# DavidHan008/SLAM-1

Measured on AMD Instinct MI355X. Metric: frames/sec tracking+local-BA @1280x720, higher is better.
Workload: dtype u8+f32+f64

## Files before the change

### include/slam355.h

```cpp
#ifndef SLAM355_H
#define SLAM355_H

#include <stddef.h>
#include <stdint.h>

#ifdef __cplusplus
extern "C" {
#endif

#define SLAM355_ABI_VERSION 1

#define SLAM_OK 0
#define SLAM_ERR_ARG (-1)
#define SLAM_ERR_HIP (-2)
#define SLAM_ERR_WORKSPACE (-3)
#define SLAM_ERR_COMM (-4)

int slam_abi_version(void);
const char* slam_last_error(void);
int slam_device_count(void);

int slam_hamming_knn2(const uint8_t* d_q, const int32_t* d_nq, int q_cap,
                      const uint8_t* d_t, const int32_t* d_nt, int t_cap,
                      int batch, int32_t* d_idx2, int32_t* d_dist2,
                      uint8_t* d_good, void* stream);

int slam_hamming_force_valu(int valu);

int slam_compact_matches(const int32_t* d_idx2, const uint8_t* d_good,
                         const int32_t* d_nq, int q_cap, int batch,
                         const double* d_gate_xyz, double gate,
                         int32_t* d_pairs, int32_t* d_count, void* stream);



int slam_gather_matches(const float* d_kpq, int kq_cap, const float* d_kpt, int kt_cap,
                        const uint8_t* d_desq, const uint8_t* d_dest, const int32_t* d_pairs,
                        const int32_t* d_count, int p_cap, int batch, double* d_ptq,
                        double* d_ptt, uint8_t* d_dq, uint8_t* d_dt, void* stream);

int slam_gather_temporal(const double* d_X, const double* d_ptl, int xcap, const float* d_kp_next,
                         int kcap, const int32_t* d_pairs, const int32_t* d_count, int pcap,
                         int batch, double* d_Q1, double* d_q2, double* d_q1, void* stream);

int slam_fundamental_lmeds(const double* d_m1, const double* d_m2, const int32_t* d_count,
                           int cap, int batch, uint64_t seed, int item0, int n_hyp,
                           uint8_t* d_mask, double* d_F, int32_t* d_ninliers, void* stream);

int slam_filter_pairs(const int32_t* d_pairs, const int32_t* d_count, const uint8_t* d_mask,
                      int cap, int batch, int32_t* d_out, int32_t* d_out_count, void* stream);

int slam_triangulate(const double* d_ptl, const double* d_ptr, const int32_t* d_count, int cap,
                     int batch, const double* d_Pl, const double* d_Pr, int proj_stride,
                     double* d_X, void* stream);

int slam_pnp_ransac(const double* d_Q, const double* d_q, const int32_t* d_count, int cap,
                    int batch, const double* d_K, uint64_t seed, int item0, int n_hyp,
                    double reproj_thresh, int hyp_iters, int refine_iters, double* d_rvec,
                    double* d_tvec, int32_t* d_ninliers, uint8_t* d_mask, double* d_ws,
                    long long ws_len, void* stream);
long long slam_pnp_workspace_len(int batch, int n_hyp);

int slam_pose_chain(const double* d_rvec, const double* d_tvec, const int32_t* d_ninliers,
                    int batch, double* d_state, double* d_poses, void* stream);

int slam_vo_estimate_pose(const double* d_q1, const double* d_q2, const double* d_Q1,
                          const double* d_Q2, const int32_t* d_count, int cap, int batch,
                          const double* d_P, uint64_t seed, int item0, int max_iter,
                          int lm_iters, int early_stop, double* d_pose, int32_t* d_best,
                          int32_t* d_ntried, double* d_err, void* d_ws, size_t ws_bytes,
                          void* stream);
int slam_vo_pose_workspace_bytes(int batch, int max_iter, size_t* bytes);

int slam_vo_residuals(const double* d_dof, const double* d_q1, const double* d_q2,
                      const double* d_Q1, const double* d_Q2, const int32_t* d_count, int cap,
                      int batch, const double* d_P, double* d_res, void* stream);

int slam_rel_to_abs(const double* d_rel, const int32_t* d_count, int cap, int batch,
                    const double* d_poses, double* d_abs, void* stream);

int slam_map_workspace_bytes(int max_queries, int map_cap, size_t* bytes);
int slam_map_associate(double* d_map, int32_t* d_M, int map_cap, int M_bound,
                       const double* d_abs, const double* d_rel, const double* d_pts2d,
                       const int32_t* d_n, int N, double threshold, int frame_index,
                       double* d_rows, void* d_ws, size_t ws_size, void* stream);
int slam_map_windows(double* d_maps, int32_t* d_M, int map_cap, int n_win, int n,
                     const double* d_abs, const double* d_rel, const double* d_pts2d,
                     const int32_t* d_count, int cap, double threshold, double* d_rows,
                     void* d_ws, size_t ws_size, void* stream);

int slam_orb_workspace_bytes(int batch, int H, int W, int max_kp, int overlap_div,
                             int height_div, int width_div, size_t* bytes);
int slam_orb_tiles(const uint8_t* d_img, int batch, int H, int W, int stride, int max_kp,
                   int overlap_div, int height_div, int width_div, void* d_ws,
                   size_t ws_bytes, float* d_kp, int32_t* d_octave, uint8_t* d_desc,
                   int32_t* d_count, int kp_cap, void* stream);


int slam_ba_residual(const double* d_cams, const double* d_pts, const int32_t* d_cam_idx,
                     const int32_t* d_pt_idx, const double* d_qs, int n_obs,
// ... 194 lines not shown
```

### slam-1_amd/csrc/fundamental.hip

```cpp
#include "common.hpp"

#include <cmath>

namespace {

#ifndef SLAM_FMH_WG
#define SLAM_FMH_WG 256
#endif
constexpr int kHWG = SLAM_FMH_WG, kHWaves = kHWG / 64;
constexpr int kFWG = 64;
constexpr int kS = 7;

__device__ inline uint64_t splitmix64(uint64_t& s) {
  s += 0x9E3779B97F4A7C15ull;
  uint64_t z = s;
  z = (z ^ (z >> 30)) * 0xBF58476D1CE4E5B9ull;
  z = (z ^ (z >> 27)) * 0x94D049BB133111EBull;
  return z ^ (z >> 31);
}

__device__ __forceinline__ void draw_sample(uint64_t& s, int M, int idx[kS]) {
#pragma unroll
  for (int k = 0; k < kS; ++k) {
    int v;
// ... 188 lines not shown
  const double cc2 = (v1 + vm) / 2.0 - cc0;
  const double s = (v1 - vm) / 2.0;
  const double u = v2 - 4.0 * cc2 - cc0;
  const double cc3 = (u - 2.0 * s) / 6.0;
  const double cc1 = s - cc3;
  double roots[3];
  const int nr = cubic_roots(cc3, cc2, cc1, cc0, roots);
  const double T1[9] = {s1, 0, -s1 * c1x, 0, s1, -s1 * c1y, 0, 0, 1};
  const double T2[9] = {s2, 0, -s2 * c2x, 0, s2, -s2 * c2y, 0, 0, 1};
  int n = 0;
#pragma unroll
  for (int k = 0; k < 3; ++k) {
    if (k >= nr) break;
    double Fn[9], tmp[9], F[9];
#pragma unroll
    for (int i = 0; i < 9; ++i) Fn[i] = roots[k] * F1[i] + (1.0 - roots[k]) * F2[i];
#pragma unroll
    for (int i = 0; i < 3; ++i)
#pragma unroll
      for (int j = 0; j < 3; ++j)
        tmp[3 * i + j] = Fn[3 * i] * T1[j] + Fn[3 * i + 1] * T1[3 + j] + Fn[3 * i + 2] * T1[6 + j];
#pragma unroll
    for (int i = 0; i < 3; ++i)
#pragma unroll
      for (int j = 0; j < 3; ++j)
        F[3 * i + j] = T2[i] * tmp[j] + T2[3 + i] * tmp[3 + j] + T2[6 + i] * tmp[6 + j];
    double nrm = 0.0;
#pragma unroll
    for (int i = 0; i < 9; ++i) nrm += F[i] * F[i];
    nrm = sqrt(nrm);
    if (!(nrm > 0.0) || !isfinite(nrm)) continue;
#pragma unroll
    for (int i = 0; i < 9; ++i) out[n][i] = F[i] / nrm;
    ++n;
  }
  return n;
}

__device__ __forceinline__ float fm_error(const double* F, const double* p1, const double* p2) {
  double a = F[0] * p1[0] + F[1] * p1[1] + F[2];
  double b = F[3] * p1[0] + F[4] * p1[1] + F[5];
  double c = F[6] * p1[0] + F[7] * p1[1] + F[8];
  const double s2 = 1.0 / (a * a + b * b);
  const double d2 = p2[0] * a + p2[1] * b + c;
  a = F[0] * p2[0] + F[3] * p2[1] + F[6];
  b = F[1] * p2[0] + F[4] * p2[1] + F[7];
  c = F[2] * p2[0] + F[5] * p2[1] + F[8];
  const double s1 = 1.0 / (a * a + b * b);
  const double d1 = p1[0] * a + p1[1] * b + c;
  const float e = (float)fmax(d1 * d1 * s1, d2 * d2 * s2);
  return isnan(e) ? INFINITY : e;
}

constexpr int kSplit = 8;
constexpr int kRound = 64;
constexpr int kEv = 12;
static_assert(kSplit * 8 <= 9 * 8, "per-split bests must fit F[b]");
#ifdef SLAM_FMH_TRACE
__device__ unsigned long long g_fmh[8];
#define FMH_T(i) do { if (threadIdx.x == 0 && blockIdx.x == 3 && blockIdx.y == 5) g_fmh[i] = __builtin_amdgcn_s_memtime(); } while (0)
#else
#define FMH_T(i) (void)0
#endif

__global__ __launch_bounds__(kHWG) void k_fm_hyp(const double* __restrict__ m1all,
                                                const double* __restrict__ m2all,
                                                const int32_t* __restrict__ count, int cap,
                                                uint64_t seed, int item0, int n_hyp,
                                                double* __restrict__ Fout) {
  __shared__ double cand[kRound][3][9];
  __shared__ int ncand[kRound];
  __shared__ int hist[kHWaves][256];
  __shared__ float wbest[kHWaves];
  __shared__ int wbidx[kHWaves];
  const int b = blockIdx.x, sp = blockIdx.y, t = threadIdx.x;
  const int lane = t & 63, w = t >> 6;
  const int M = min(max(count[b], 0), cap);
  if (M < 8) return;
  const double* m1 = m1all + (size_t)b * cap * 2;
  const double* m2 = m2all + (size_t)b * cap * 2;
  const int hb = (int)((long long)n_hyp * sp / kSplit), he = (int)((long long)n_hyp * (sp + 1) / kSplit);
  float my_best = INFINITY;
  int my_idx = 0x7FFFFFFF;
  const int need = M / 2 + 1;
  FMH_T(0);
#ifdef SLAM_FMH_TRACE
  int n_sel = 0, n_cand = 0;
#endif
  for (int h0 = hb; h0 < he; h0 += kRound) {
    const int nh = min(kRound, he - h0);
    __syncthreads();
    if (t < nh) {
      const int h = h0 + t;
      uint64_t s = seed ^ ((uint64_t)(item0 + b) * 0xD1B54A32D192ED03ull) ^
                   ((uint64_t)h * 0x9FB21C651E98DF25ull);
      int idx[kS];
      draw_sample(s, M, idx);
      ncand[t] = seven_point(m1, m2, idx, cand[t]);
    }
    __syncthreads();
    FMH_T(1);
    int ln = lane;
    asm volatile("" : "+v"(ln));
    double pc[kEv][4];
#pragma unroll
    for (int j = 0; j < kEv; ++j) {
      const int i = min(ln + 64 * j, M - 1);
      pc[j][0] = m1[2 * i];
      pc[j][1] = m1[2 * i + 1];
      pc[j][2] = m2[2 * i];
      pc[j][3] = m2[2 * i + 1];
    }
    for (int hl = w; hl < nh; hl += kHWaves) {
      for (int k = 0; k < ncand[hl]; ++k) {
        const double* F = cand[hl][k];
        int below = 0;
        float ev[kEv];
#pragma unroll
        for (int j = 0; j < kEv; ++j) {
          ev[j] = INFINITY;
          if (ln + 64 * j < M) {
            ev[j] = fm_error(F, pc[j], pc[j] + 2);
            below += ev[j] < my_best ? 1 : 0;
          }
        }
        for (int i = ln + 64 * kEv; i < M; i += 64)
          below += fm_error(F, m1 + 2 * i, m2 + 2 * i) < my_best ? 1 : 0;
        for (int off = 32; off > 0; off >>= 1) below += __shfl_xor(below, off, 64);
#ifdef SLAM_FMH_TRACE
        ++n_cand;
#endif
        if (below < need) continue;
#ifdef SLAM_FMH_TRACE
        ++n_sel;
#endif
        uint32_t prefix = 0, pmask = 0;
        int krank = M / 2;
        for (int shift = 24; shift >= 0; shift -= 8) {
          for (int j = lane; j < 256; j += 64) hist[w][j] = 0;
          __builtin_amdgcn_wave_barrier();
#pragma unroll
          for (int j = 0; j < kEv; ++j) {
            const uint32_t bits = __float_as_uint(ev[j]);
            if (ln + 64 * j < M && (bits & pmask) == prefix)
              atomicAdd(&hist[w][(bits >> shift) & 255u], 1);
          }
          for (int i = ln + 64 * kEv; i < M; i += 64) {
            const uint32_t bits = __float_as_uint(fm_error(F, m1 + 2 * i, m2 + 2 * i));
            if ((bits & pmask) == prefix) atomicAdd(&hist[w][(bits >> shift) & 255u], 1);
          }
          __builtin_amdgcn_wave_barrier();
          __builtin_amdgcn_s_waitcnt(0xC07F);
          const int c0 = hist[w][4 * lane], c1 = hist[w][4 * lane + 1];
          const int c2 = hist[w][4 * lane + 2], c3 = hist[w][4 * lane + 3];
          const int sm = c0 + c1 + c2 + c3;
          int inc = sm;
          for (int off = 1; off < 64; off <<= 1) {
            const int o = __shfl_up(inc, off, 64);
            if (lane >= off) inc += o;
          }
          const int exc = inc - sm;
          int bin = -1, before = 0;
          if (krank >= exc && krank < inc) {
            int acc = exc;
            if (krank < acc + c0) { bin = 4 * lane; before = acc; }
            else if (krank < acc + c0 + c1) { bin = 4 * lane + 1; before = acc + c0; }
            else if (krank < acc + c0 + c1 + c2) { bin = 4 * lane + 2; before = acc + c0 + c1; }
            else { bin = 4 * lane + 3; before = acc + c0 + c1 + c2; }
          }
          const unsigned long long bal = __ballot(bin >= 0);
          const int src = __ffsll((long long)bal) - 1;
          bin = __shfl(bin, src, 64);
          before = __shfl(before, src, 64);
          krank -= before;
          prefix |= (uint32_t)bin << shift;
          pmask |= 255u << shift;
        }
        const float med = __uint_as_float(prefix);
        if (med < my_best) {
          my_best = med;
          my_idx = (h0 + hl) * 3 + k;
        }
      }
    }
  }
  FMH_T(2);
#ifdef SLAM_FMH_TRACE
  if (threadIdx.x == 0 && blockIdx.x == 3 && blockIdx.y == 5) { g_fmh[5] = n_cand; g_fmh[6] = n_sel; g_fmh[7] = M; }
#endif
  if (lane == 0) {
    wbest[w] = my_best;
    wbidx[w] = my_idx;
  }
  __syncthreads();
  FMH_T(3);
  if (t == 0) {
    float bm = INFINITY;
    int bi = 0x7FFFFFFF;
    for (int i = 0; i < kHWaves; ++i)
      if (wbest[i] < bm || (wbest[i] == bm && wbidx[i] < bi)) {
        bm = wbest[i];
        bi = wbidx[i];
      }
    float* slot = reinterpret_cast<float*>(Fout + 9 * (size_t)b) + 2 * sp;
    slot[0] = bm;
    reinterpret_cast<int*>(slot)[1] = bi;
  }
}

__global__ __launch_bounds__(kFWG) void k_fm_finish(const double* __restrict__ m1all,
                                                   const double* __restrict__ m2all,
                                                   const int32_t* __restrict__ count, int cap,
                                                   uint64_t seed, int item0,
                                                   uint8_t* __restrict__ mask,
                                                   double* __restrict__ Fout,
                                                   int32_t* __restrict__ ninl) {
  __shared__ double Fb[9];
  __shared__ double Fw[3][9];
  __shared__ float best_s;
  __shared__ int found_s, cnt_s;
  const int b = blockIdx.x, t = threadIdx.x;
  const int lane = t & 63;
  const int M = min(max(count[b], 0), cap);
  const double* m1 = m1all + (size_t)b * cap * 2;
  const double* m2 = m2all + (size_t)b * cap * 2;
  uint8_t* mk = mask + (size_t)b * cap;
  if (M < 8) {
    for (int i = t; i < M; i += kFWG) mk[i] = 0;
    if (t < 9) Fout[9 * b + t] = 0.0;
    if (t == 0) ninl[b] = -1;
    return;
  }
  if (t == 0) {
    const float* slots = reinterpret_cast<const float*>(Fout + 9 * (size_t)b);
    float bm = INFINITY;
    int bi = 0x7FFFFFFF;
    for (int i = 0; i < kSplit; ++i) {
      const float v = slots[2 * i];
      const int ix = reinterpret_cast<const int*>(slots)[2 * i + 1];
      if (v < bm || (v == bm && ix < bi)) {
        bm = v;
        bi = ix;
      }
    }
    best_s = bm;
    found_s = bi != 0x7FFFFFFF && bm < INFINITY;
    cnt_s = 0;
    if (found_s) {
      const int h = bi / 3, k = bi % 3;
      uint64_t s = seed ^ ((uint64_t)(item0 + b) * 0xD1B54A32D192ED03ull) ^
                   ((uint64_t)h * 0x9FB21C651E98DF25ull);
      int idx[kS];
      draw_sample(s, M, idx);
      seven_point(m1, m2, idx, Fw);
      for (int i = 0; i < 9; ++i) Fb[i] = Fw[k][i];
    }
  }
  __syncthreads();
  if (!found_s) {
    for (int i = t; i < M; i += kFWG) mk[i] = 0;
    if (t < 9) Fout[9 * b + t] = 0.0;
    if (t == 0) ninl[b] = -1;
    return;
  }
  double sigma = 2.5 * 1.4826 * (1 + 5.0 / (M - kS)) * sqrt((double)best_s);
  sigma = fmax(sigma, 0.001);
  const double thr = sigma * sigma;
  double F[9];
  for (int i = 0; i < 9; ++i) F[i] = Fb[i];
  int c = 0;
  for (int i = t; i < M; i += kFWG) {
    const uint8_t in = (double)fm_error(F, m1 + 2 * i, m2 + 2 * i) <= thr ? 1 : 0;
    mk[i] = in;
    c += in;
  }
  for (int off = 32; off > 0; off >>= 1) c += __shfl_xor(c, off, 64);
  if (lane == 0) atomicAdd(&cnt_s, c);
  __syncthreads();
  if (t < 9) Fout[9 * b + t] = F[t];
  if (t == 0) ninl[b] = cnt_s;
}

#ifndef SLAM_CWG
#define SLAM_CWG 1024
#endif
constexpr int kCWG = SLAM_CWG;
__global__ __launch_bounds__(kCWG) void k_filter_pairs(const int2* __restrict__ pairs,
                                                       const int32_t* __restrict__ count,
                                                       const uint8_t* __restrict__ mask, int cap,
                                                       int2* __restrict__ out,
                                                       int32_t* __restrict__ out_count) {
  __shared__ int wave_tot[kCWG / 64];
  __shared__ int carry;
  const int b = blockIdx.x;
  const int n = min(max(count[b], 0), cap);
  const int lane = threadIdx.x & 63, wid = threadIdx.x >> 6;
  if (threadIdx.x == 0) carry = 0;
  __syncthreads();
  for (int base = 0; base < n; base += kCWG) {
    const int k = base + threadIdx.x;
    const bool keep = k < n && mask[(size_t)b * cap + k] != 0;
    const unsigned long long m = __ballot(keep);
    const int before = __popcll(m & ((1ull << lane) - 1ull));
    if (lane == 0) wave_tot[wid] = __popcll(m);
    __syncthreads();
    int off = carry;
    for (int i = 0; i < wid; ++i) off += wave_tot[i];
    if (keep) out[(size_t)b * cap + off + before] = pairs[(size_t)b * cap + k];
    __syncthreads();
    if (threadIdx.x == 0) {
      int tot = 0;
      for (int i = 0; i < kCWG / 64; ++i) tot += wave_tot[i];
      carry += tot;
    }
    __syncthreads();
  }
  if (threadIdx.x == 0) out_count[b] = carry;
}

}

extern "C" int slam_fundamental_lmeds(const double* d_m1, const double* d_m2,
                                      const int32_t* d_count, int cap, int batch, uint64_t seed,
                                      int item0, int n_hyp, uint8_t* d_mask, double* d_F,
                                      int32_t* d_ninliers, void* stream) {
  SLAM_REQUIRE(batch >= 0 && cap >= 0, "slam_fundamental_lmeds: bad shape");
  SLAM_REQUIRE(n_hyp >= 1 && n_hyp <= 4096, "slam_fundamental_lmeds: n_hyp in [1, 4096]");
  if (batch == 0) return SLAM_OK;
  SLAM_REQUIRE(d_m1 && d_m2 && d_count && d_mask && d_F && d_ninliers,
               "slam_fundamental_lmeds: null pointer");
  hipStream_t s = slam::as_stream(stream);
  k_fm_hyp<<<dim3(batch, kSplit), kHWG, 0, s>>>(d_m1, d_m2, d_count, cap, seed, item0, n_hyp, d_F);
  SLAM_LAUNCHED("k_fm_hyp");
  k_fm_finish<<<batch, kFWG, 0, s>>>(d_m1, d_m2, d_count, cap, seed, item0, d_mask, d_F,
                                    d_ninliers);
  SLAM_LAUNCHED("k_fm_finish");
  return SLAM_OK;
}

extern "C" int slam_filter_pairs(const int32_t* d_pairs, const int32_t* d_count,
                                 const uint8_t* d_mask, int cap, int batch, int32_t* d_out,
                                 int32_t* d_out_count, void* stream) {
  SLAM_REQUIRE(batch >= 0 && cap >= 0, "slam_filter_pairs: bad shape");
  if (batch == 0) return SLAM_OK;
  SLAM_REQUIRE(d_pairs && d_count && d_mask && d_out && d_out_count,
               "slam_filter_pairs: null pointer");
  SLAM_REQUIRE(d_out != d_pairs, "slam_filter_pairs: in-place filtering is not supported");
  k_filter_pairs<<<batch, kCWG, 0, slam::as_stream(stream)>>>(
      reinterpret_cast<const int2*>(d_pairs), d_count, d_mask, cap, reinterpret_cast<int2*>(d_out),
      d_out_count);
  SLAM_LAUNCHED("k_filter_pairs");
  return SLAM_OK;
}

#ifdef SLAM_FMH_TRACE
extern "C" int slam_fmh_trace(unsigned long long* out) {
  SLAM_HIP(hipDeviceSynchronize());
  SLAM_HIP(hipMemcpyFromSymbol(out, HIP_SYMBOL(g_fmh), 8 * sizeof(unsigned long long)));
  return SLAM_OK;
}
#endif
```

### slam-1_amd/slam355/_lib.py

```python
from __future__ import annotations

import ctypes
import os

_HERE = os.path.dirname(os.path.abspath(__file__))
LIB_PATH = os.environ.get("SLAM355_LIB") or os.path.join(_HERE, "libslam355.so")

c_int = ctypes.c_int
c_double = ctypes.c_double
c_size_t = ctypes.c_size_t
c_p = ctypes.c_void_p
c_uint64 = ctypes.c_uint64
c_longlong = ctypes.c_longlong

c_i32 = ctypes.c_int32


class BAProblemStruct(ctypes.Structure):
    _fields_ = [
        ("n_cams", c_i32), ("n_pts", c_i32), ("n_obs", c_i32), ("n_grps", c_i32),
        ("n_blocks", c_i32), ("n_cslots", c_i32), ("n_bslots", c_i32), ("lin_mode", c_i32),
        ("n_sgrps", c_i32), ("tl_mode", c_i32),
        ("cams", c_p * 2), ("pts", c_p * 2), ("camrec", c_p * 2),
        ("obs_cam", c_p), ("obs_pt", c_p), ("obs_q", c_p), ("pt_ptr", c_p), ("grp_ptr", c_p),
# ... 6 lines not shown
        ("sg_ptr", c_p), ("sg_meta", c_p), ("obs_meta", c_p), ("chk_optr", c_p), ("chk_cptr", c_p),
        ("bslot_ab", c_p), ("tl_sched", c_p), ("tl_sched_host", c_p), ("asm_tab", c_p),
        ("asm_act", c_p), ("n_asm_act", c_int), ("asm_pad", c_int),
    ]


_PROB = ctypes.POINTER(BAProblemStruct)

PLAN_TABLES = ("perm", "order", "obs_cam", "obs_pt", "pt_ptr", "grp_ptr", "grp_cslot", "cslot_cam",
               "grp_bslot", "bslot_blk", "blocks", "cam_cslot_ptr", "cslot_row", "blk_bslot_ptr",
               "bslot_row", "sg_ptr", "sg_meta", "sg_cams", "obs_la", "chk_cobs", "obs_meta",
               "chk_optr", "chk_cptr", "bslot_ab")


class PlanInfo(ctypes.Structure):
    _fields_ = [
        ("ok", c_i32), ("n_obs", c_i32), ("n_grps", c_i32), ("n_sgrps", c_i32),
        ("n_cslots", c_i32), ("n_bslots", c_i32), ("n_blocks", c_i32), ("chunks_per_wg", c_i32),
        ("off", ctypes.c_longlong * len(PLAN_TABLES)), ("len", ctypes.c_longlong * len(PLAN_TABLES)),
        ("total", ctypes.c_longlong),
    ]

SIGNATURES = {
    "slam_abi_version": [],
    "slam_last_error": [],
    "slam_device_count": [],
    "slam_hamming_knn2": [c_p, c_p, c_int, c_p, c_p, c_int, c_int, c_p, c_p, c_p, c_p],
    "slam_compact_matches": [c_p, c_p, c_p, c_int, c_int, c_p, c_double, c_p, c_p, c_p],
    "slam_orb_workspace_bytes": [c_int, c_int, c_int, c_int, c_int, c_int, c_int,
                                 ctypes.POINTER(c_size_t)],
    "slam_orb_tiles": [c_p, c_int, c_int, c_int, c_int, c_int, c_int, c_int, c_int, c_p,
                       c_size_t, c_p, c_p, c_p, c_p, c_int, c_p],
    "slam_gather_matches": [c_p, c_int, c_p, c_int, c_p, c_p, c_p, c_p, c_int, c_int, c_p, c_p,
                            c_p, c_p, c_p],
    "slam_gather_temporal": [c_p, c_p, c_int, c_p, c_int, c_p, c_p, c_int, c_int, c_p, c_p, c_p,
                             c_p],
    "slam_triangulate": [c_p, c_p, c_p, c_int, c_int, c_p, c_p, c_int, c_p, c_p],
    "slam_pnp_ransac": [c_p, c_p, c_p, c_int, c_int, c_p, c_uint64, c_int, c_int, c_double, c_int,
                        c_int, c_p, c_p, c_p, c_p, c_p, c_longlong, c_p],
    "slam_pnp_workspace_len": [c_int, c_int],
    "slam_pose_chain": [c_p, c_p, c_p, c_int, c_p, c_p, c_p],
    "slam_vo_estimate_pose": [c_p, c_p, c_p, c_p, c_p, c_int, c_int, c_p, c_uint64, c_int, c_int,
                              c_int, c_int, c_p, c_p, c_p, c_p, c_p, c_size_t, c_p],
    "slam_vo_pose_workspace_bytes": [c_int, c_int, ctypes.POINTER(c_size_t)],
    "slam_vo_residuals": [c_p, c_p, c_p, c_p, c_p, c_p, c_int, c_int, c_p, c_p, c_p],
    "slam_map_workspace_bytes": [c_int, c_int, ctypes.POINTER(c_size_t)],
    "slam_rel_to_abs": [c_p, c_p, c_int, c_int, c_p, c_p, c_p],
    "slam_map_windows": [c_p, c_p, c_int, c_int, c_int, c_p, c_p, c_p, c_p, c_int, c_double, c_p,
                         c_p, c_size_t, c_p],
    "slam_map_associate": [c_p, c_p, c_int, c_int, c_p, c_p, c_p, c_p, c_int, c_double, c_int,
                           c_p, c_p, c_size_t, c_p],
    "slam_fundamental_lmeds": [c_p, c_p, c_p, c_int, c_int, c_uint64, c_int, c_int, c_p, c_p, c_p,
                               c_p],
    "slam_filter_pairs": [c_p, c_p, c_p, c_int, c_int, c_p, c_p, c_p],
    "slam_ba_residual": [c_p, c_p, c_p, c_p, c_p, c_int, c_p, c_p],
    "slam_ba_jacobian": [c_p, c_p, c_p, c_p, c_p, c_int, c_p, c_p, c_p],
    "slam_ba_red_slots": [c_int],
    "slam_ba_sys_len": [c_int, c_int],
    "slam_ba_chol_len": [c_int, c_p],
    "slam_ba_build_system": [_PROB, c_p],
    "slam_ba_solve_step": [_PROB, c_p],
    "slam_ba_decide": [_PROB, c_p],
    "slam_ba_iterate": [_PROB, c_int, c_p],
    "slam_ba_reset": [_PROB, c_double, c_p],
    "slam_ba_iterate_batch": [_PROB, c_int, c_int, c_p],
    "slam_ba_set_solve_lds_floor": [c_int],
    "slam_orb_set_lds_floor": [c_int],
    "slam_count_min": [c_p, c_int, c_p, c_p],
    "slam_hamming_force_valu": [c_int],
    "slam_ba_reset_batch": [_PROB, c_int, c_double, c_p],
    "slam_pose_chain_objective": [c_p, c_int, c_int, c_int, c_p, c_p],
    "slam_bow_histograms": [c_p, c_p, c_int, c_int, c_int, c_p, c_int, c_p, c_p, c_p],
    "slam_bow_query": [c_p, c_int, c_p, c_p, c_int, c_p, c_p, c_p],
    "slam_bow_lloyd": [c_p, c_int, c_p, c_p, c_int, c_int, c_p, c_p, c_p],
    "slam_pose_chain_workspace_len": [c_int],
    "slam_fast_tiles_workspace_bytes": [c_int, c_int, c_int, c_int, c_int, c_int,
                                        ctypes.POINTER(c_size_t)],
    "slam_fast_tiles": [c_p, c_int, c_int, c_int, c_int, c_int, c_int, c_int, c_int, c_p,
                        c_size_t, c_p, c_p, c_int, c_p],
    "slam_lk_pyramid_layout": [c_int, c_int, c_int, c_int, ctypes.POINTER(c_int),
                               ctypes.POINTER(c_size_t)],
    "slam_lk_build_pyramids": [c_p, c_int, c_int, c_int, c_int, c_int, c_int, c_p, c_p, c_p],
    "slam_lk_track": [c_p, c_p, c_p, ctypes.c_longlong, c_int, c_int, c_int, c_int, c_int, c_int,
                      c_double, ctypes.c_float, c_p, c_int, c_p, c_int, c_p, c_p, c_p, c_p],
    "slam_lk_filter": [c_p, c_int, c_p, c_p, c_p, c_p, c_int, c_int, c_int, c_int, ctypes.c_float,
                       c_int, c_p, c_p, c_p, c_p, c_p],
    "slam_sgbm_workspace_bytes": [c_int, c_int, c_int, c_int, c_int, c_int,
                                  ctypes.POINTER(c_size_t)],
    "slam_sgbm": [c_p, c_p, c_int, c_int, c_int, c_int, c_int, c_int, c_int, c_int, c_int, c_p,
                  c_size_t, c_p, c_p, c_p],
    "slam_vo_right_qs_3d": [c_p, c_p, c_p, c_int, c_int, c_p, ctypes.c_longlong,
                            ctypes.c_longlong, c_int, c_int, ctypes.c_float, ctypes.c_float, c_p,
                            c_p, c_p, c_p, c_p, c_p, c_p, c_p, c_p, c_p, c_p, c_p, c_p, c_p],
    "slam_triangulate_f32": [c_p, c_p, c_p, c_int, c_int, c_p, c_p, c_p, c_p],
    "slam_pose_chain_trf": [c_p, c_int, c_int, c_int, c_int, c_double, c_double, c_double, c_int,
                            c_p, c_p],
    "slam_comm_unique_id": [c_p],
    "slam_comm_init": [c_int, c_int, c_p, ctypes.POINTER(c_p)],
    "slam_comm_destroy": [c_p],
    "slam_comm_allreduce_f64": [c_p, c_p, ctypes.c_longlong, c_p],
    "slam_ba_step_distributed": [_PROB, c_p, c_p],
    "slam_ba_plan_bound": [c_int, c_int, c_int, c_int],
    "slam_ba_plan_mfma": [c_int, c_int, c_int, c_p, c_p, c_p, c_int, c_int, c_p, c_longlong,
                          ctypes.POINTER(PlanInfo)],
    "slam_ba_stage_windows": [c_int, c_int, c_int, c_p, c_p, c_p, c_int, c_p, c_p, c_double,
                              c_double, c_p, c_longlong, c_p, c_longlong, c_p, c_p, c_p, c_p, c_p],
}
_RESTYPE = {"slam_last_error": ctypes.c_char_p, "slam_ba_sys_len": ctypes.c_longlong,
            "slam_ba_plan_bound": ctypes.c_longlong,
            "slam_ba_chol_len": ctypes.c_longlong, "slam_pnp_workspace_len": ctypes.c_longlong, "slam_pose_chain_workspace_len": ctypes.c_longlong}


class SlamError(RuntimeError):
    """A libslam355 call returned a non-zero status."""


def _load():
    if not os.path.exists(LIB_PATH):
        raise ImportError(
            f"libslam355.so not found at {LIB_PATH}: build it with "
            "`make -C slam-1_amd` (or __graft_entry__.build()). slam355 has no CPU fallback."
        )
    import torch

    lib = ctypes.CDLL(LIB_PATH)
    for name, argtypes in SIGNATURES.items():
        fn = getattr(lib, name)
        fn.argtypes = argtypes
        fn.restype = _RESTYPE.get(name, c_int)
    return lib


lib = _load()


def check(rc: int, what: str = "") -> None:
    if rc != 0:
        msg = lib.slam_last_error().decode(errors="replace")
        raise SlamError(f"{what or 'libslam355'} failed ({rc}): {msg}")


def call(name: str, *args) -> None:
    check(getattr(lib, name)(*args), name)
```

### slam-1_amd/slam355/geometry.py

```python
from __future__ import annotations

import ctypes

import numpy as np
import torch

from . import _lib
from .device import ptr, require_gpu, stream_ptr

PNP_DEFAULTS = dict(n_hyp=100, reproj_thresh=8.0, hyp_iters=10, refine_iters=20)


def gather_matches(kpq, kpt, pairs, count, desq=None, dest=None, out=None, stream=None):
    B, p_cap, _ = pairs.shape
    dev = pairs.device
    if out is None:
        ptq = torch.zeros((B, p_cap, 2), dtype=torch.float64, device=dev)
        ptt = torch.zeros((B, p_cap, 2), dtype=torch.float64, device=dev)
        dq = dt = None
        if desq is not None:
            dq = torch.zeros((B, p_cap, 32), dtype=torch.uint8, device=dev)
            dt = torch.zeros((B, p_cap, 32), dtype=torch.uint8, device=dev)
    else:
        ptq, ptt, dq, dt = out
    _lib.call("slam_gather_matches", ptr(kpq), kpq.shape[1], ptr(kpt), kpt.shape[1], ptr(desq),
              ptr(dest), ptr(pairs), ptr(count), p_cap, B, ptr(ptq), ptr(ptt), ptr(dq), ptr(dt),
              stream_ptr(stream))
    return ptq, ptt, dq, dt


def gather_temporal(X, ptl, kp_next, pairs, count, out=None, stream=None):
    B, pcap, _ = pairs.shape
    dev = pairs.device
    if out is None:
        Q1 = torch.zeros((B, pcap, 3), dtype=torch.float64, device=dev)
        q2 = torch.zeros((B, pcap, 2), dtype=torch.float64, device=dev)
        q1 = torch.zeros((B, pcap, 2), dtype=torch.float64, device=dev)
    else:
        Q1, q2, q1 = out
    _lib.call("slam_gather_temporal", ptr(X), ptr(ptl), X.shape[1], ptr(kp_next), kp_next.shape[1],
              ptr(pairs), ptr(count), pcap, B, ptr(Q1), ptr(q2), ptr(q1), stream_ptr(stream))
    return Q1, q2, q1


def fundamental_lmeds(m1, m2, count, seed=0, item0=0, n_hyp=300, out=None, stream=None):
    B, cap, _ = m1.shape
    dev = m1.device
    if out is None:
        mask = torch.zeros((B, max(cap, 1)), dtype=torch.uint8, device=dev)
        F = torch.zeros((B, 9), dtype=torch.float64, device=dev)
        ninl = torch.zeros((B,), dtype=torch.int32, device=dev)
    else:
        mask, F, ninl = out
    _lib.call("slam_fundamental_lmeds", ptr(m1), ptr(m2), ptr(count), cap, B,
              int(seed) & ((1 << 64) - 1), int(item0), int(n_hyp), ptr(mask), ptr(F), ptr(ninl),
              stream_ptr(stream))
    return mask, F, ninl


def filter_pairs(pairs, count, mask, out=None, stream=None):
    B, cap, _ = pairs.shape
    if out is None:
        o = torch.empty_like(pairs)
        oc = torch.empty((B,), dtype=torch.int32, device=pairs.device)
    else:
        o, oc = out
    _lib.call("slam_filter_pairs", ptr(pairs), ptr(count), ptr(mask), cap, B, ptr(o), ptr(oc),
              stream_ptr(stream))
    return o, oc


def triangulate(ptl, ptr_, count, P_l, P_r, out=None, stream=None):
    B, cap, _ = ptl.shape
    Pl = P_l if isinstance(P_l, torch.Tensor) else torch.as_tensor(np.asarray(P_l, np.float64),
                                                                   device=ptl.device)
    Pr = P_r if isinstance(P_r, torch.Tensor) else torch.as_tensor(np.asarray(P_r, np.float64),
                                                                   device=ptl.device)
    Pl, Pr = Pl.contiguous(), Pr.contiguous()
    stride = 12 if Pl.dim() == 3 else 0
    X = out if out is not None else torch.zeros((B, cap, 3), dtype=torch.float64, device=ptl.device)
    _lib.call("slam_triangulate", ptr(ptl), ptr(ptr_), ptr(count), cap, B, ptr(Pl), ptr(Pr), stride,
              ptr(X), stream_ptr(stream))
    return X


def pnp_ransac(Q, q, count, K, seed=0, item0=0, out=None, stream=None, ws=None, **kw):
    prm = dict(PNP_DEFAULTS, **kw)
    B, cap, _ = Q.shape
    dev = Q.device
    Kt = K if isinstance(K, torch.Tensor) else torch.as_tensor(np.asarray(K, np.float64), device=dev)
    if out is None:
        rvec = torch.zeros((B, 3), dtype=torch.float64, device=dev)
        tvec = torch.zeros((B, 3), dtype=torch.float64, device=dev)
        ninl = torch.zeros((B,), dtype=torch.int32, device=dev)
        mask = torch.zeros((B, max(cap, 1)), dtype=torch.uint8, device=dev)
    else:
        rvec, tvec, ninl, mask = out
    if ws is None:
        ws = pnp_workspace(B, prm["n_hyp"], dev)
        if stream is not None and stream != torch.cuda.current_stream(dev):
            ws.record_stream(stream)
    _lib.call("slam_pnp_ransac", ptr(Q), ptr(q), ptr(count), cap, B, ptr(Kt.contiguous()),
              int(seed) & ((1 << 64) - 1), int(item0), prm["n_hyp"], float(prm["reproj_thresh"]),
              prm["hyp_iters"], prm["refine_iters"], ptr(rvec), ptr(tvec), ptr(ninl), ptr(mask),
              ptr(ws), ws.numel(), stream_ptr(stream))
    return rvec, tvec, ninl, mask


def pnp_workspace(B, n_hyp=PNP_DEFAULTS["n_hyp"], dev="cuda"):
    n = int(_lib.lib.slam_pnp_workspace_len(B, n_hyp))
# ... 38 lines not shown
```

### slam-1_amd/slam355/pipeline.py

```python
from __future__ import annotations

import time

import numpy as np
import torch

from . import _lib, geometry, matcher, orb
from .device import ptr, require_gpu, stream_ptr


class Tracker:

    def __init__(self, B, H, W, P_l, P_r, max_kp_per_tile=56, seed=0, max_distance=500.0,
                 stream=None, orb_stream=None):
        self.dev = require_gpu()
        self.B, self.H, self.W = B, H, W
        self.max_kp = max_kp_per_tile
        self.seed = seed
        self.max_distance = float(max_distance)
        self.stream = stream
        self.P_l = np.asarray(P_l, np.float64)
        self.P_r = np.asarray(P_r, np.float64)
        self.K = self.P_l[:3, :3].copy()
        d = self.dev
        self.tPl = torch.as_tensor(self.P_l, device=d).contiguous()
        self.tPr = torch.as_tensor(self.P_r, device=d).contiguous()
        self.tK = torch.as_tensor(self.K, device=d).contiguous()
        self.ows = orb.OrbWorkspace(2 * B + 1, H, W, max_kp_per_tile)
        self.orb_stream = orb_stream
        if orb_stream is not None:
            self.ows_pair = [self.ows, orb.OrbWorkspace(2 * B + 1, H, W, max_kp_per_tile)]
            self.orb_done = [torch.cuda.Event() for _ in range(2)]
            self.slot_free = [torch.cuda.Event() for _ in range(2)]
            self._k = 0
        cap = self.cap = self.ows.kp_cap
        i32 = dict(dtype=torch.int32, device=d)
        f64 = dict(dtype=torch.float64, device=d)
        u8 = dict(dtype=torch.uint8, device=d)
        self.s_idx2 = torch.full((B, cap, 2), -1, **i32)
        self.s_dist2 = torch.full((B, cap, 2), -1, **i32)
        self.s_good = torch.zeros((B, cap), **u8)
        self.s_pairs = torch.zeros((B, cap, 2), **i32)
        self.s_cnt = torch.zeros((B,), **i32)
        self.s_ptl = torch.zeros((B, cap, 2), **f64)
        self.s_ptr = torch.zeros((B, cap, 2), **f64)
        self.f_mask = torch.zeros((B, cap), **u8)
        self.f_F = torch.zeros((B, 9), **f64)
        self.f_ninl = torch.zeros((B,), **i32)
        self.f_pairs = torch.zeros((B, cap, 2), **i32)
        self.f_cnt = torch.zeros((B,), **i32)
        self.f_ptl = torch.zeros((B, cap, 2), **f64)
        self.f_ptr = torch.zeros((B, cap, 2), **f64)
        self.f_dl = torch.zeros((B, cap, 32), **u8)
        self.f_dr = torch.zeros((B, cap, 32), **u8)
        self.X = torch.zeros((B, cap, 3), **f64)
        self.t_idx2 = torch.full((B, cap, 2), -1, **i32)
        self.t_dist2 = torch.full((B, cap, 2), -1, **i32)
        self.t_good = torch.zeros((B, cap), **u8)
        self.t_pairs = torch.zeros((B, cap, 2), **i32)
        self.t_cnt = torch.zeros((B,), **i32)
        self.Q1 = torch.zeros((B, cap, 3), **f64)
        self.q2 = torch.zeros((B, cap, 2), **f64)
        self.q1 = torch.zeros((B, cap, 2), **f64)
        self.rvec = torch.zeros((B, 3), **f64)
        self.tvec = torch.zeros((B, 3), **f64)
        self.p_ninl = torch.zeros((B,), **i32)
        self.p_mask = torch.zeros((B, cap), **u8)
        self.p_ws = geometry.pnp_workspace(B, dev=d)
        self.imgs = torch.zeros((2 * B + 1, H, W), **u8)
        self.chain_state = torch.zeros((32,), **f64)
        self._chain_eye = torch.from_numpy(np.concatenate([np.eye(4), np.eye(4)]).ravel()).to(d)
        self.reset_chain()
        self.poses = torch.zeros((B, 4, 4), **f64)
        self.orb_min = torch.full((1,), 1 << 30, **i32)
        self.orb_event = torch.cuda.Event()
        self.host_times = None

    def _ht(self, site, t0):
        t1 = time.perf_counter()
        if self.host_times is not None:
            self.host_times.setdefault(site, []).append(t1 - t0)
        return t1

    def track(self, frame0: int, imgs: torch.Tensor | None = None, marks=None, chain=True):
        B, st = self.B, self.stream
        im = self.imgs if imgs is None else imgs

        def mark(name):
            if marks is not None:
                ev = torch.cuda.Event(enable_timing=True)
                ev.record(st if st is not None else torch.cuda.current_stream())
                marks.append((name, ev))

        main = st if st is not None else torch.cuda.current_stream()
        ost = self.orb_stream
        h0 = time.perf_counter()
        if ost is None:
            mark("start")
            kp, octv, desc, cnt = self.ows.run(im, st)
            _lib.call("slam_count_min", ptr(cnt), cnt.numel(), ptr(self.orb_min), stream_ptr(main))
            self.orb_event.record(main)
            mark("orb")
        else:
            slot = self._k % 2
            self._k += 1
            self.ows = ows = self.ows_pair[slot]
            ost.wait_event(self.slot_free[slot])
            if imgs is None:
                ost.wait_stream(main)
            if marks is not None:
                e0 = torch.cuda.Event(enable_timing=True)
                e0.record(ost)
            kp, octv, desc, cnt = ows.run(im, ost)
            _lib.call("slam_count_min", ptr(cnt), cnt.numel(), ptr(self.orb_min), stream_ptr(ost))
            if marks is not None:
                e1 = torch.cuda.Event(enable_timing=True)
                e1.record(ost)
                self.orb_marks = [("start", e0), ("orb", e1)]
            self.orb_event.record(ost)
            self.orb_done[slot].record(ost)
            main.wait_event(self.orb_done[slot])
            mark("orb_wait")
        h0 = self._ht("orb_launch", h0)
        kpL, kpR = kp[0:B], kp[B + 1:2 * B + 1]
        dL, dR = desc[0:B], desc[B + 1:2 * B + 1]
        nL, nR = cnt[0:B], cnt[B + 1:2 * B + 1]
        kpL1, dL1, nL1 = kp[1:B + 1], desc[1:B + 1], cnt[1:B + 1]
        matcher.knn2_batch(dL, nL, dR, nR, out=(self.s_idx2, self.s_dist2, self.s_good), stream=st)
        mark("stereo_knn2")
        matcher.compact_matches(self.s_idx2, self.s_good, nL, out=(self.s_pairs, self.s_cnt),
                                stream=st)
        geometry.gather_matches(kpL, kpR, self.s_pairs, self.s_cnt,
                                out=(self.s_ptl, self.s_ptr, None, None), stream=st)
        mark("stereo_match")
        h0 = self._ht("stereo_launch", h0)
        geometry.fundamental_lmeds(self.s_ptl, self.s_ptr, self.s_cnt, seed=self.seed,
                                   item0=frame0, out=(self.f_mask, self.f_F, self.f_ninl),
                                   stream=st)
        mark("f_lmeds")
        geometry.filter_pairs(self.s_pairs, self.s_cnt, self.f_mask,
                              out=(self.f_pairs, self.f_cnt), stream=st)
        geometry.gather_matches(kpL, kpR, self.f_pairs, self.f_cnt, dL, dR,
                                out=(self.f_ptl, self.f_ptr, self.f_dl, self.f_dr), stream=st)
        geometry.triangulate(self.f_ptl, self.f_ptr, self.f_cnt, self.tPl, self.tPr, out=self.X,
                             stream=st)
        matcher.knn2_batch(self.f_dl, self.f_cnt, dL1, nL1,
                           out=(self.t_idx2, self.t_dist2, self.t_good), stream=st)
        matcher.compact_matches(self.t_idx2, self.t_good, self.f_cnt, gate_xyz=self.X,
                                gate=self.max_distance, out=(self.t_pairs, self.t_cnt), stream=st)
        geometry.gather_temporal(self.X, self.f_ptl, kpL1, self.t_pairs, self.t_cnt,
                                 out=(self.Q1, self.q2, self.q1), stream=st)
        if ost is not None:
            self.slot_free[slot].record(main)
        mark("triangulate_temporal")
        h0 = self._ht("flmeds_tri_temporal_launch", h0)
        geometry.pnp_ransac(self.Q1, self.q2, self.t_cnt, self.tK, seed=self.seed, item0=frame0,
                            out=(self.rvec, self.tvec, self.p_ninl, self.p_mask), stream=st,
                            ws=self.p_ws)
        mark("pnp")
        h0 = self._ht("pnp_launch", h0)
        if chain:
            _lib.call("slam_pose_chain", ptr(self.rvec), ptr(self.tvec), ptr(self.p_ninl), B,
                      ptr(self.chain_state), ptr(self.poses), stream_ptr(st))
            mark("pose_chain")
            self._ht("pose_chain_launch", h0)
        return self.rvec, self.tvec, self.p_ninl

    def reset_chain(self, pose0=None, T0=None):
        with torch.cuda.stream(self.stream if self.stream is not None
                               else torch.cuda.current_stream()):
            if pose0 is None and T0 is None:
                src = self._chain_eye
            else:
                st = np.concatenate([np.eye(4) if pose0 is None else np.asarray(pose0, float),
                                     np.eye(4) if T0 is None else np.asarray(T0, float)]).ravel()
                src = torch.from_numpy(st).to(self.chain_state.device)
            self.chain_state.copy_(src, non_blocking=True)

    def check(self):
        cur = torch.cuda.current_stream()
        streams = [x for x in (self.stream, self.orb_stream) if x is not None]
        for x in streams:
            cur.wait_stream(x)
        m = int(self.orb_min.item())
        self.orb_min.fill_(1 << 30)
        for x in streams:
            x.wait_stream(cur)
        if m < 0:
            raise _lib.SlamError("Tracker: ORB keypoint workspace overflow (a tile kept more tied "
                                 "responses than the workspace holds, or kp_cap was exceeded); "
                                 "the frame would have been tracked with no matches")
# ... 149 lines not shown
```

Measured before the change: 22120.

## Split fundamental LMedS into separate hypothesis-solve and LDS-staged scoring kernels

Moves seven-point hypothesis generation out of the scoring kernel into its own fully parallel kernel that writes candidate F matrices to a workspace. The scoring kernel now reads candidates from the workspace and stages match points in LDS instead of register-caching them per round. The finish kernel also reads the winning F from the workspace rather than recomputing it. This removes the serialized per-round solve and its block barriers, at the cost of an extra launch, workspace traffic and a preallocated buffer.

New measurement: 22410 (median of 6 runs). 1.3% higher.

```diff
diff --git a/include/slam355.h b/include/slam355.h
--- a/include/slam355.h
+++ b/include/slam355.h
@@ -46,6 +46,11 @@
 int slam_fundamental_lmeds(const double* d_m1, const double* d_m2, const int32_t* d_count,
                            int cap, int batch, uint64_t seed, int item0, int n_hyp,
                            uint8_t* d_mask, double* d_F, int32_t* d_ninliers, void* stream);
+int slam_fundamental_lmeds_ws(const double* d_m1, const double* d_m2, const int32_t* d_count,
+                              int cap, int batch, uint64_t seed, int item0, int n_hyp,
+                              uint8_t* d_mask, double* d_F, int32_t* d_ninliers, double* d_ws,
+                              long long ws_len, void* stream);
+long long slam_fundamental_workspace_len(int batch, int n_hyp);
 
 int slam_filter_pairs(const int32_t* d_pairs, const int32_t* d_count, const uint8_t* d_mask,
                       int cap, int batch, int32_t* d_out, int32_t* d_out_count, void* stream);
diff --git a/slam-1_amd/csrc/fundamental.hip b/slam-1_amd/csrc/fundamental.hip
--- a/slam-1_amd/csrc/fundamental.hip
+++ b/slam-1_amd/csrc/fundamental.hip
@@ -264,10 +264,32 @@
   return isnan(e) ? INFINITY : e;
 }
 
+constexpr int kRec = 28;
+constexpr int kSWG = 64;
+
+__global__ __launch_bounds__(kSWG) void k_fm_solve(const double* __restrict__ m1all,
+                                                  const double* __restrict__ m2all,
+                                                  const int32_t* __restrict__ count, int cap,
+                                                  uint64_t seed, int item0, int n_hyp,
+                                                  double* __restrict__ ws) {
+  const int b = blockIdx.y, h = blockIdx.x * kSWG + threadIdx.x;
+  const int M = min(max(count[b], 0), cap);
+  if (M < 8 || h >= n_hyp) return;
+  const double* m1 = m1all + (size_t)b * cap * 2;
+  const double* m2 = m2all + (size_t)b * cap * 2;
+  uint64_t s = seed ^ ((uint64_t)(item0 + b) * 0xD1B54A32D192ED03ull) ^
+               ((uint64_t)h * 0x9FB21C651E98DF25ull);
+  int idx[kS];
+  draw_sample(s, M, idx);
+  double* rec = ws + ((size_t)b * n_hyp + h) * kRec;
+  rec[0] = (double)seven_point(m1, m2, idx, reinterpret_cast<double (*)[9]>(rec + 1));
+}
+
 constexpr int kSplit = 8;
-constexpr int kRound = 64;
 constexpr int kEv = 12;
+constexpr int kLdsPts = 1024;
 static_assert(kSplit * 8 <= 9 * 8, "per-split bests must fit F[b]");
+static_assert(kLdsPts >= 64 * kEv, "the register-cached errors cover staged points first");
 #ifdef SLAM_FMH_TRACE
 __device__ unsigned long long g_fmh[8];
 #define FMH_T(i) do { if (threadIdx.x == 0 && blockIdx.x == 3 && blockIdx.y == 5) g_fmh[i] = __builtin_amdgcn_s_memtime(); } while (0)
@@ -275,126 +297,138 @@
 #define FMH_T(i) (void)0
 #endif
 
-__global__ __launch_bounds__(kHWG) void k_fm_hyp(const double* __restrict__ m1all,
-                                                const double* __restrict__ m2all,
-                                                const int32_t* __restrict__ count, int cap,
-                                                uint64_t seed, int item0, int n_hyp,
-                                                double* __restrict__ Fout) {
-  __shared__ double cand[kRound][3][9];
-  __shared__ int ncand[kRound];
+struct PtsLds {
+  const double2* p1;
+  const double2* p2;
+  __device__ __forceinline__ float error(const double* F, int i) const {
+    const double2 a = p1[i], c = p2[i];
+    const double u[2] = {a.x, a.y}, v[2] = {c.x, c.y};
+    return fm_error(F, u, v);
+  }
+};
+struct PtsGlobal {
+  const double* m1;
+  const double* m2;
+  __device__ __forceinline__ float error(const double* F, int i) const {
+    return fm_error(F, m1 + 2 * i, m2 + 2 * i);
+  }
+};
+
+template <class Pts>
+__device__ __forceinline__ void fm_score_range(const Pts& pts, const double* __restrict__ recs,
+                                               int hb, int he, int w, int lane, int M, int* hist,
+                                               float& my_best, int& my_idx, int& n_cand,
+                                               int& n_sel) {
+  const int need = M / 2 + 1;
+  for (int h = hb + w; h < he; h += kHWaves) {
+    const double* rec = recs + (size_t)h * kRec;
+    const int nc = (int)rec[0];
+    for (int k = 0; k < nc; ++k) {
+      double F[9];
+#pragma unroll
+      for (int i = 0; i < 9; ++i) F[i] = rec[1 + 9 * k + i];
+      int ln = lane;
+      asm volatile("" : "+v"(ln));
+      int below = 0;
+      float ev[kEv];
+#pragma unroll
+      for (int j = 0; j < kEv; ++j) {
+        ev[j] = INFINITY;
+        if (ln + 64 * j < M) {
+          ev[j] = pts.error(F, ln + 64 * j);
+          below += ev[j] < my_best ? 1 : 0;
+        }
+      }
+      for (int i = ln + 64 * kEv; i < M; i += 64) below += pts.error(F, i) < my_best ? 1 : 0;
+      for (int off = 32; off > 0; off >>= 1) below += __shfl_xor(below, off, 64);
+      ++n_cand;
+      if (below < need) continue;
+      ++n_sel;
+      uint32_t prefix = 0, pmask = 0;
+      int krank = M / 2;
+      for (int shift = 24; shift >= 0; shift -= 8) {
+        for (int j = lane; j < 256; j += 64) hist[j] = 0;
+        __builtin_amdgcn_wave_barrier();
+#pragma unroll
+        for (int j = 0; j < kEv; ++j) {
+          const uint32_t bits = __float_as_uint(ev[j]);
+          if (ln + 64 * j < M && (bits & pmask) == prefix)
+            atomicAdd(&hist[(bits >> shift) & 255u], 1);
+        }
+        for (int i = ln + 64 * kEv; i < M; i += 64) {
+          const uint32_t bits = __float_as_uint(pts.error(F, i));
+          if ((bits & pmask) == prefix) atomicAdd(&hist[(bits >> shift) & 255u], 1);
+        }
+        __builtin_amdgcn_wave_barrier();
+        __builtin_amdgcn_s_waitcnt(0xC07F);
+        const int c0 = hist[4 * lane], c1 = hist[4 * lane + 1];
+        const int c2 = hist[4 * lane + 2], c3 = hist[4 * lane + 3];
+        const int sm = c0 + c1 + c2 + c3;
+        int inc = sm;
+        for (int off = 1; off < 64; off <<= 1) {
+          const int o = __shfl_up(inc, off, 64);
+          if (lane >= off) inc += o;
+        }
+        const int exc = inc - sm;
+        int bin = -1, before = 0;
+        if (krank >= exc && krank < inc) {
+          int acc = exc;
+          if (krank < acc + c0) { bin = 4 * lane; before = acc; }
+          else if (krank < acc + c0 + c1) { bin = 4 * lane + 1; before = acc + c0; }
+          else if (krank < acc + c0 + c1 + c2) { bin = 4 * lane + 2; before = acc + c0 + c1; }
+          else { bin = 4 * lane + 3; before = acc + c0 + c1 + c2; }
+        }
+        const unsigned long long bal = __ballot(bin >= 0);
+        const int src = __ffsll((long long)bal) - 1;
+        bin = __shfl(bin, src, 64);
+        before = __shfl(before, src, 64);
+        krank -= before;
+        prefix |= (uint32_t)bin << shift;
+        pmask |= 255u << shift;
+      }
+      const float med = __uint_as_float(prefix);
+      if (med < my_best) {
+        my_best = med;
+        my_idx = h * 3 + k;
+      }
+    }
+  }
+}
+
+__global__ __launch_bounds__(kHWG, 4) void k_fm_score(const double* __restrict__ m1all,
+                                                  const double* __restrict__ m2all,
+                                                  const int32_t* __restrict__ count, int cap,
+                                                  int n_hyp, const double* __restrict__ ws,
+                                                  double* __restrict__ Fout) {
+  __shared__ double2 sp1[kLdsPts], sp2[kLdsPts];
   __shared__ int hist[kHWaves][256];
   __shared__ float wbest[kHWaves];
   __shared__ int wbidx[kHWaves];
   const int b = blockIdx.x, sp = blockIdx.y, t = threadIdx.x;
-  const int lane = t & 63, w = t >> 6;
+  const int lane = t & 63, w = __builtin_amdgcn_readfirstlane(t >> 6);
   const int M = min(max(count[b], 0), cap);
   if (M < 8) return;
   const double* m1 = m1all + (size_t)b * cap * 2;
   const double* m2 = m2all + (size_t)b * cap * 2;
+  const double* recs = ws + (size_t)b * n_hyp * kRec;
   const int hb = (int)((long long)n_hyp * sp / kSplit), he = (int)((long long)n_hyp * (sp + 1) / kSplit);
   float my_best = INFINITY;
   int my_idx = 0x7FFFFFFF;
-  const int need = M / 2 + 1;
+  int n_cand = 0, n_sel = 0;
   FMH_T(0);
-#ifdef SLAM_FMH_TRACE
-  int n_sel = 0, n_cand = 0;
-#endif
-  for (int h0 = hb; h0 < he; h0 += kRound) {
-    const int nh = min(kRound, he - h0);
-    __syncthreads();
-    if (t < nh) {
-      const int h = h0 + t;
-      uint64_t s = seed ^ ((uint64_t)(item0 + b) * 0xD1B54A32D192ED03ull) ^
-                   ((uint64_t)h * 0x9FB21C651E98DF25ull);
-      int idx[kS];
-      draw_sample(s, M, idx);
-      ncand[t] = seven_point(m1, m2, idx, cand[t]);
+  if (M <= kLdsPts) {
+    for (int i = t; i < M; i += kHWG) {
+      sp1[i] = make_double2(m1[2 * i], m1[2 * i + 1]);
+      sp2[i] = make_double2(m2[2 * i], m2[2 * i + 1]);
     }
     __syncthreads();
     FMH_T(1);
-    int ln = lane;
-    asm volatile("" : "+v"(ln));
-    double pc[kEv][4];
-#pragma unroll
-    for (int j = 0; j < kEv; ++j) {
-      const int i = min(ln + 64 * j, M - 1);
-      pc[j][0] = m1[2 * i];
-      pc[j][1] = m1[2 * i + 1];
-      pc[j][2] = m2[2 * i];
-      pc[j][3] = m2[2 * i + 1];
-    }
-    for (int hl = w; hl < nh; hl += kHWaves) {
-      for (int k = 0; k < ncand[hl]; ++k) {
-        const double* F = cand[hl][k];
-        int below = 0;
-        float ev[kEv];
-#pragma unroll
-        for (int j = 0; j < kEv; ++j) {
-          ev[j] = INFINITY;
-          if (ln + 64 * j < M) {
-            ev[j] = fm_error(F, pc[j], pc[j] + 2);
-            below += ev[j] < my_best ? 1 : 0;
-          }
-        }
-        for (int i = ln + 64 * kEv; i < M; i += 64)
-          below += fm_error(F, m1 + 2 * i, m2 + 2 * i) < my_best ? 1 : 0;
-        for (int off = 32; off > 0; off >>= 1) below += __shfl_xor(below, off, 64);
-#ifdef SLAM_FMH_TRACE
-        ++n_cand;
-#endif
-        if (below < need) continue;
-#ifdef SLAM_FMH_TRACE
-        ++n_sel;
-#endif
-        uint32_t prefix = 0, pmask = 0;
-        int krank = M / 2;
-        for (int shift = 24; shift >= 0; shift -= 8) {
-          for (int j = lane; j < 256; j += 64) hist[w][j] = 0;
-          __builtin_amdgcn_wave_barrier();
-#pragma unroll
-          for (int j = 0; j < kEv; ++j) {
-            const uint32_t bits = __float_as_uint(ev[j]);
-            if (ln + 64 * j < M && (bits & pmask) == prefix)
-              atomicAdd(&hist[w][(bits >> shift) & 255u], 1);
-          }
-          for (int i = ln + 64 * kEv; i < M; i += 64) {
-            const uint32_t bits = __float_as_uint(fm_error(F, m1 + 2 * i, m2 + 2 * i));
-            if ((bits & pmask) == prefix) atomicAdd(&hist[w][(bits >> shift) & 255u], 1);
-          }
-          __builtin_amdgcn_wave_barrier();
-          __builtin_amdgcn_s_waitcnt(0xC07F);
-          const int c0 = hist[w][4 * lane], c1 = hist[w][4 * lane + 1];
-          const int c2 = hist[w][4 * lane + 2], c3 = hist[w][4 * lane + 3];
-          const int sm = c0 + c1 + c2 + c3;
-          int inc = sm;
-          for (int off = 1; off < 64; off <<= 1) {
-            const int o = __shfl_up(inc, off, 64);
-            if (lane >= off) inc += o;
-          }
-          const int exc = inc - sm;
-          int bin = -1, before = 0;
-          if (krank >= exc && krank < inc) {
-            int acc = exc;
-            if (krank < acc + c0) { bin = 4 * lane; before = acc; }
-            else if (krank < acc + c0 + c1) { bin = 4 * lane + 1; before = acc + c0; }
-            else if (krank < acc + c0 + c1 + c2) { bin = 4 * lane + 2; before = acc + c0 + c1; }
-            else { bin = 4 * lane + 3; before = acc + c0 + c1 + c2; }
-          }
-          const unsigned long long bal = __ballot(bin >= 0);
-          const int src = __ffsll((long long)bal) - 1;
-          bin = __shfl(bin, src, 64);
-          before = __shfl(before, src, 64);
-          krank -= before;
-          prefix |= (uint32_t)bin << shift;
-          pmask |= 255u << shift;
-        }
-        const float med = __uint_as_float(prefix);
-        if (med < my_best) {
-          my_best = med;
-          my_idx = (h0 + hl) * 3 + k;
-        }
-      }
-    }
+    fm_score_range(PtsLds{sp1, sp2}, recs, hb, he, w, lane, M, hist[w], my_best, my_idx, n_cand,
+                   n_sel);
+  } else {
+    FMH_T(1);
+    fm_score_range(PtsGlobal{m1, m2}, recs, hb, he, w, lane, M, hist[w], my_best, my_idx, n_cand,
+                   n_sel);
   }
   FMH_T(2);
 #ifdef SLAM_FMH_TRACE
@@ -423,14 +457,12 @@
 __global__ __launch_bounds__(kFWG) void k_fm_finish(const double* __restrict__ m1all,
                                                    const double* __restrict__ m2all,
                                                    const int32_t* __restrict__ count, int cap,
-                                                   uint64_t seed, int item0,
+                                                   int n_hyp, const double* __restrict__ ws,
                                                    uint8_t* __restrict__ mask,
                                                    double* __restrict__ Fout,
                                                    int32_t* __restrict__ ninl) {
-  __shared__ double Fb[9];
-  __shared__ double Fw[3][9];
   __shared__ float best_s;
-  __shared__ int found_s, cnt_s;
+  __shared__ int found_s, bidx_s, cnt_s;
   const int b = blockIdx.x, t = threadIdx.x;
   const int lane = t & 63;
   const int M = min(max(count[b], 0), cap);
@@ -457,16 +489,8 @@
     }
     best_s = bm;
     found_s = bi != 0x7FFFFFFF && bm < INFINITY;
+    bidx_s = bi;
     cnt_s = 0;
-    if (found_s) {
-      const int h = bi / 3, k = bi % 3;
-      uint64_t s = seed ^ ((uint64_t)(item0 + b) * 0xD1B54A32D192ED03ull) ^
-                   ((uint64_t)h * 0x9FB21C651E98DF25ull);
-      int idx[kS];
-      draw_sample(s, M, idx);
-      seven_point(m1, m2, idx, Fw);
-      for (int i = 0; i < 9; ++i) Fb[i] = Fw[k][i];
-    }
   }
   __syncthreads();
   if (!found_s) {
@@ -478,8 +502,10 @@
   double sigma = 2.5 * 1.4826 * (1 + 5.0 / (M - kS)) * sqrt((double)best_s);
   sigma = fmax(sigma, 0.001);
   const double thr = sigma * sigma;
+  const int bi = bidx_s;
+  const double* Fw = ws + ((size_t)b * n_hyp + bi / 3) * kRec + 1 + 9 * (bi % 3);
   double F[9];
-  for (int i = 0; i < 9; ++i) F[i] = Fb[i];
+  for (int i = 0; i < 9; ++i) F[i] = Fw[i];
   int c = 0;
   for (int i = t; i < M; i += kFWG) {
     const uint8_t in = (double)fm_error(F, m1 + 2 * i, m2 + 2 * i) <= thr ? 1 : 0;
@@ -532,6 +558,35 @@
 
 }
 
+extern "C" long long slam_fundamental_workspace_len(int batch, int n_hyp) {
+  return (long long)(batch > 0 ? batch : 0) * (n_hyp > 0 ? n_hyp : 0) * kRec;
+}
+
+extern "C" int slam_fundamental_lmeds_ws(const double* d_m1, const double* d_m2,
+                                         const int32_t* d_count, int cap, int batch,
+                                         uint64_t seed, int item0, int n_hyp, uint8_t* d_mask,
+                                         double* d_F, int32_t* d_ninliers, double* d_ws,
+                                         long long ws_len, void* stream) {
+  SLAM_REQUIRE(batch >= 0 && cap >= 0, "slam_fundamental_lmeds_ws: bad shape");
+  SLAM_REQUIRE(n_hyp >= 1 && n_hyp <= 4096, "slam_fundamental_lmeds_ws: n_hyp in [1, 4096]");
+  SLAM_REQUIRE(ws_len >= slam_fundamental_workspace_len(batch, n_hyp),
+               "slam_fundamental_lmeds_ws: workspace %lld < %lld doubles", ws_len,
+               slam_fundamental_workspace_len(batch, n_hyp));
+  if (batch == 0) return SLAM_OK;
+  SLAM_REQUIRE(d_m1 && d_m2 && d_count && d_mask && d_F && d_ninliers && d_ws,
+               "slam_fundamental_lmeds_ws: null pointer");
+  hipStream_t s = slam::as_stream(stream);
+  k_fm_solve<<<dim3((n_hyp + kSWG - 1) / kSWG, batch), kSWG, 0, s>>>(d_m1, d_m2, d_count, cap, seed,
+                                                                    item0, n_hyp, d_ws);
+  SLAM_LAUNCHED("k_fm_solve");
+  k_fm_score<<<dim3(batch, kSplit), kHWG, 0, s>>>(d_m1, d_m2, d_count, cap, n_hyp, d_ws, d_F);
+  SLAM_LAUNCHED("k_fm_score");
+  k_fm_finish<<<batch, kFWG, 0, s>>>(d_m1, d_m2, d_count, cap, n_hyp, d_ws, d_mask, d_F,
+                                    d_ninliers);
+  SLAM_LAUNCHED("k_fm_finish");
+  return SLAM_OK;
+}
+
 extern "C" int slam_fundamental_lmeds(const double* d_m1, const double* d_m2,
                                       const int32_t* d_count, int cap, int batch, uint64_t seed,
                                       int item0, int n_hyp, uint8_t* d_mask, double* d_F,
@@ -542,12 +597,13 @@
   SLAM_REQUIRE(d_m1 && d_m2 && d_count && d_mask && d_F && d_ninliers,
                "slam_fundamental_lmeds: null pointer");
   hipStream_t s = slam::as_stream(stream);
-  k_fm_hyp<<<dim3(batch, kSplit), kHWG, 0, s>>>(d_m1, d_m2, d_count, cap, seed, item0, n_hyp, d_F);
-  SLAM_LAUNCHED("k_fm_hyp");
-  k_fm_finish<<<batch, kFWG, 0, s>>>(d_m1, d_m2, d_count, cap, seed, item0, d_mask, d_F,
-                                    d_ninliers);
-  SLAM_LAUNCHED("k_fm_finish");
-  return SLAM_OK;
+  const long long n = slam_fundamental_workspace_len(batch, n_hyp);
+  double* ws = nullptr;
+  SLAM_HIP(hipMallocAsync(reinterpret_cast<void**>(&ws), (size_t)n * sizeof(double), s));
+  const int rc = slam_fundamental_lmeds_ws(d_m1, d_m2, d_count, cap, batch, seed, item0, n_hyp,
+                                           d_mask, d_F, d_ninliers, ws, n, s);
+  SLAM_HIP(hipFreeAsync(ws, s));
+  return rc;
 }
 
 extern "C" int slam_filter_pairs(const int32_t* d_pairs, const int32_t* d_count,
diff --git a/slam-1_amd/slam355/_lib.py b/slam-1_amd/slam355/_lib.py
--- a/slam-1_amd/slam355/_lib.py
+++ b/slam-1_amd/slam355/_lib.py
@@ -82,6 +82,9 @@
                            c_p, c_p, c_size_t, c_p],
     "slam_fundamental_lmeds": [c_p, c_p, c_p, c_int, c_int, c_uint64, c_int, c_int, c_p, c_p, c_p,
                                c_p],
+    "slam_fundamental_lmeds_ws": [c_p, c_p, c_p, c_int, c_int, c_uint64, c_int, c_int, c_p, c_p,
+                                  c_p, c_p, c_longlong, c_p],
+    "slam_fundamental_workspace_len": [c_int, c_int],
     "slam_filter_pairs": [c_p, c_p, c_p, c_int, c_int, c_p, c_p, c_p],
     "slam_ba_residual": [c_p, c_p, c_p, c_p, c_p, c_int, c_p, c_p],
     "slam_ba_jacobian": [c_p, c_p, c_p, c_p, c_p, c_int, c_p, c_p, c_p],
@@ -138,7 +141,9 @@
 }
 _RESTYPE = {"slam_last_error": ctypes.c_char_p, "slam_ba_sys_len": ctypes.c_longlong,
             "slam_ba_plan_bound": ctypes.c_longlong,
-            "slam_ba_chol_len": ctypes.c_longlong, "slam_pnp_workspace_len": ctypes.c_longlong, "slam_pose_chain_workspace_len": ctypes.c_longlong}
+            "slam_ba_chol_len": ctypes.c_longlong, "slam_pnp_workspace_len": ctypes.c_longlong,
+            "slam_fundamental_workspace_len": ctypes.c_longlong,
+            "slam_pose_chain_workspace_len": ctypes.c_longlong}
 
 
 class SlamError(RuntimeError):
diff --git a/slam-1_amd/slam355/geometry.py b/slam-1_amd/slam355/geometry.py
--- a/slam-1_amd/slam355/geometry.py
+++ b/slam-1_amd/slam355/geometry.py
@@ -43,7 +43,7 @@
     return Q1, q2, q1
 
 
-def fundamental_lmeds(m1, m2, count, seed=0, item0=0, n_hyp=300, out=None, stream=None):
+def fundamental_lmeds(m1, m2, count, seed=0, item0=0, n_hyp=300, out=None, stream=None, ws=None):
     B, cap, _ = m1.shape
     dev = m1.device
     if out is None:
@@ -52,10 +52,18 @@
         ninl = torch.zeros((B,), dtype=torch.int32, device=dev)
     else:
         mask, F, ninl = out
-    _lib.call("slam_fundamental_lmeds", ptr(m1), ptr(m2), ptr(count), cap, B,
-              int(seed) & ((1 << 64) - 1), int(item0), int(n_hyp), ptr(mask), ptr(F), ptr(ninl),
-              stream_ptr(stream))
+    args = (ptr(m1), ptr(m2), ptr(count), cap, B, int(seed) & ((1 << 64) - 1), int(item0),
+            int(n_hyp), ptr(mask), ptr(F), ptr(ninl))
+    if ws is None:
+        _lib.call("slam_fundamental_lmeds", *args, stream_ptr(stream))
+    else:
+        _lib.call("slam_fundamental_lmeds_ws", *args, ptr(ws), ws.numel(), stream_ptr(stream))
     return mask, F, ninl
+
+
+def fundamental_workspace(B, n_hyp=300, dev="cuda"):
+    n = int(_lib.lib.slam_fundamental_workspace_len(B, n_hyp))
+    return torch.empty(max(n, 1), dtype=torch.float64, device=dev)
 
 
 def filter_pairs(pairs, count, mask, out=None, stream=None):
diff --git a/slam-1_amd/slam355/pipeline.py b/slam-1_amd/slam355/pipeline.py
--- a/slam-1_amd/slam355/pipeline.py
+++ b/slam-1_amd/slam355/pipeline.py
@@ -67,6 +67,7 @@
         self.p_ninl = torch.zeros((B,), **i32)
         self.p_mask = torch.zeros((B, cap), **u8)
         self.p_ws = geometry.pnp_workspace(B, dev=d)
+        self.f_ws = geometry.fundamental_workspace(B, dev=d)
         self.imgs = torch.zeros((2 * B + 1, H, W), **u8)
         self.chain_state = torch.zeros((32,), **f64)
         self._chain_eye = torch.from_numpy(np.concatenate([np.eye(4), np.eye(4)]).ravel()).to(d)
@@ -136,7 +137,7 @@
         h0 = self._ht("stereo_launch", h0)
         geometry.fundamental_lmeds(self.s_ptl, self.s_ptr, self.s_cnt, seed=self.seed,
                                    item0=frame0, out=(self.f_mask, self.f_F, self.f_ninl),
-                                   stream=st)
+                                   stream=st, ws=self.f_ws)
         mark("f_lmeds")
         geometry.filter_pairs(self.s_pairs, self.s_cnt, self.f_mask,
                               out=(self.f_pairs, self.f_cnt), stream=st)
```
